# mingfeisun/DeepMimic_mujoco

Hardware: AMD Instinct MI355X
Metric: env-steps/sec (higher is better)
Workload: dtype f64

## Files before the change

deepmimic_mujoco_amd/csrc/slot_kernel.h:

```cpp
#pragma once

#include <cstddef>

#include "env_kernel.h"

namespace dm {

constexpr int SLOTS = 4, SW = 16;
#ifndef DM_SLOT_MAXROWS
#define DM_SLOT_MAXROWS 40
#endif
constexpr int SLOT_MAXROWS = DM_SLOT_MAXROWS, SLOT_MAXLIMROWS = 16, SLOT_MAXCON = 13, SLOT_MAXFRAME = 8, SLOT_MAXCAND = 32, SLOT_BOXSLOTS = 3;
constexpr int SLOT_EXTROWS = SLOT_MAXROWS - 2 * SW;
static_assert(SLOT_EXTROWS == 8 || SLOT_EXTROWS == 0, "the partial third row set holds eight rows (or is absent)");
constexpr int PAIR_PASSES = MAXPAIR / SW;
static_assert(MAXPAIR <= 128 && NG <= 16, "a candidate word holds the pair number in 7 bits and both geom numbers in 4 bits each");
constexpr int DOF_PASSES = (NV + SW - 1) / SW, HINGE_PASSES = (NU + SW - 1) / SW, Q_PASSES = (NQ + SW - 1) / SW, ENT_PASSES = (310 + SW - 1) / SW;

#ifndef DM_SLOT_ASSUME
#define DM_SLOT_ASSUME 31
#endif
#define DM_SLOT_LANE_AT(bit, x) (((DM_SLOT_ASSUME) >> (bit)) & 1 ? dmw::launder_slot_lane(x) : dmw::launder(x))

template <class R>
// ... 815 lines not shown
      dmw::pgs_row3<2 * J + 6>(t3, tsave3, t[0], t[1], nf03, B[J + 3], U[0][J + 3], U[1][J + 3], oh[2 * J + 6]);
      if (J + 4 < next) SlotExtSweep<J + 4, R>::run(U, B, t3, tsave3, t, nf03, oh, next);
    }
  }
};
template <int I, class R>
DM_DEV void slot_assemble_lane(R* ws, const R* fy, R one) {
#pragma unroll
  for (int d = 0; d + 8 <= NV; d += 8) dmw::row_add8<I>(&ws[d], &fy[d], one);
#pragma unroll
  for (int d = NV / 8 * 8; d < NV; d++) dmw::row_fmac_old<I>(ws[d], fy[d], one);
}
template <int J, class R>
struct SlotExtAssemble {
  static DM_DEV void run(R* ws, const R* fy3, R one, int next) {
    if constexpr (J < SLOT_EXTROWS) {
      slot_assemble_lane<2 * J, R>(ws, fy3, one); slot_assemble_lane<2 * J + 2, R>(ws, fy3, one); slot_assemble_lane<2 * J + 4, R>(ws, fy3, one); slot_assemble_lane<2 * J + 6, R>(ws, fy3, one);
      if (J + 4 < next) SlotExtAssemble<J + 4, R>::run(ws, fy3, one, next);
    }
  }
};

template <class R>
DM_DEV void slot_row_setup(const DevModel<R>& M, const SlotShared<R>& s, int r, bool active, RowAcc<R>& ra, R& pos, R& margin, R& dA, R& rscale) {
  const auto& W = s.r1.rw;
  const int code = active ? W.rowi[r] : 0;
  const int type = code & 0xff;
  R w[6] = {0, 0, 0, 0, 0, 0};
  unsigned long long mplus = 0, mminus = 0;
  pos = 0; margin = 0; dA = 0; rscale = 1;
  R w7 = 0;
  if (type == ROW_LIMIT) {
    const int d = (code >> 8) & 0xff;
    w7 = ((code >> 16) & 1) ? R(1) : R(-1);
    pos = W.rowv[r]; dA = M.dof_invw[d]; mplus = 1ull << d;
  } else if (type == ROW_CONTACT) {
    const int ci = (code >> 8) & 0xff, q = (code >> 16) & 0xf, cdim = (code >> 20) & 0xf;
    const R* c = W.con[ci];
    const int cw = W.coni[ci];
    const R* fm = W.frm[(cw >> 8) & 0xff];
    const auto& rec = M.pair_rec[cw & 0xff];
    const R cmu = rec.mu, ctran = rec.tran;
    const int meta = rec.meta;
    R dir[3] = {fm[0], fm[1], fm[2]};
    if (cdim != 1) {
      const R n[3] = {fm[0], fm[1], fm[2]}, t1[3] = {fm[3], fm[4], fm[5]};
      R t2[3];
      cross3(t2, n, t1);
      const R sg = (q & 1) ? -cmu : cmu;
      const R* tg = (q >> 1) ? t2 : t1;
      dir[0] += sg * tg[0]; dir[1] += sg * tg[1]; dir[2] += sg * tg[2];
    }
    cross3(w, c, dir);
    w[3] = dir[0]; w[4] = dir[1]; w[5] = dir[2];
    pos = c[3]; margin = rec.margin;
    dA = cdim == 1 ? ctran : ctran + cmu * cmu * ctran;
    rscale = cdim == 1 ? R(1) : 2 * cmu * cmu;
    mminus = TOPO.chain[meta & 0xff]; mplus = TOPO.chain[(meta >> 8) & 0xff];
  }
  for (int r6 = 0; r6 < 6; r6++) ra.w[r6] = w[r6];
  ra.w7 = w7; ra.w8 = 0; ra.vel = 0; ra.jws = 0;
  ra.plus_lo = (unsigned)mplus; ra.plus_hi = (unsigned)(mplus >> 32); ra.minus_lo = (unsigned)mminus; ra.minus_hi = (unsigned)(mminus >> 32);
}

template <class R, int NS, bool PROF = false>
DM_DEV void slot_constraint(const DevModel<R>& M, SlotShared<R>& s, int sl_in, int lane_in, int nefc, int nmax, int& ovf, const DebugOut* dbg, long long* prof = 0) {
  const int sl = DM_SLOT_LANE_AT(4, sl_in), lane = dmw::launder(lane_in);
  long long pt0 = 0, pt1 = 0, pt_enter = 0;
  if (PROF) { pt0 = dmw::clk(); pt_enter = pt0; }
#define SLOT_STAMP(k) if constexpr (NS == 1) { DM_MARK("slot_constraint_ns1_" #k); } else if constexpr (NS == 2) { DM_MARK("slot_constraint_ns2_" #k); } else { DM_MARK("slot_constraint_ns3_" #k); } if (PROF) { pt1 = dmw::clk(); prof[k] += pt1 - pt0; pt0 = pt1; }
  constexpr bool EXT = NS == 3;
  constexpr int NF = EXT ? 2 : NS;
  constexpr int NC = 16 * NF;
  constexpr int NX = EXT ? SLOT_EXTROWS : 1;
  if constexpr (NS == 1) { DM_MARK("slot_constraint_ns1_rows"); } else if constexpr (NS == 2) { DM_MARK("slot_constraint_ns2_rows"); } else { DM_MARK("slot_constraint_ns3_rows"); }
  R y[NF + 1][NV];
  RowAcc<R> ra[NF];
  bool active[NF];
  R pos[NF], margin[NF], dA[NF], rscale[NF];
#pragma unroll
  for (int k = 0; k < NF; k++) {
    const int r = sl + 16 * k;
    active[k] = r < nefc;
    slot_row_setup(M, s, r, active[k], ra[k], pos[k], margin[k], dA[k], rscale[k]);
  }
  {
    R cur[8];
    dmw::reload_fence();
    slot_load_dof_operands<0>(cur, s);
    SlotRowStep<0, NF, R>::run(y, ra, s, cur);
  }
#pragma unroll
  for (int d = 0; d < NV; d++) y[NF][d] = s.tau[d];
  if (dbg) {
#pragma unroll
    for (int k = 0; k < NF; k++) if (active[k]) {
      double* o = dbg->out + (34 * 34 + 34 * 3 + 42 + 3) + (sl + 16 * k) * (34 + 6);
#pragma unroll
      for (int d = 0; d < NV; d++) o[d] = (double)y[k][d];
    }
  }
  SLOT_STAMP(8)
  R Rr[NF], aref[NF], f[NF];
#pragma unroll
  for (int k = 0; k < NF; k++) {
    const R imp = impedance(M, pos[k] - margin[k]);
    Rr[k] = fmax(R(DM_MINVAL), (1 - imp) * dA[k] / imp);
    if (rscale[k] != R(1)) Rr[k] = fmax(R(DM_MINVAL), rscale[k] * Rr[k]);
    aref[k] = -M.B * ra[k].vel - M.K * imp * (pos[k] - margin[k]);
    const R jar = ra[k].jws - aref[k];
    f[k] = (active[k] && jar < 0) ? -jar / Rr[k] : R(0);
  }
  slot_solve_LT<NF + 1>(y, s.r2.qLD);
#pragma unroll
  for (int d = 0; d < NV; d++) {
    const R sc = s.dsq[d];
#pragma unroll
    for (int k = 0; k <= NF; k++) { y[k][d] *= sc; dmw::pin_value(y[k][d]); }
  }
  if (dbg) {
    R x[NV];
#pragma unroll
    for (int d = 0; d < NV; d++) x[d] = y[NF][d] * s.dsq[d];
    solve_L(x, s.r2.qLD);
    if (sl == 0) {
#pragma unroll
      for (int d = 0; d < NV; d++) dbg->out[34 * 34 + 34 + d] = (double)x[d];
    }
  }
  R bb[NF];
#pragma unroll
  for (int k = 0; k < NF; k++) {
    R acc0 = 0, acc1 = 0;
#pragma unroll
    for (int d = 0; d < NV; d++) { if (d & 1) acc1 += y[k][d] * y[NF][d]; else acc0 += y[k][d] * y[NF][d]; }
    bb[k] = active[k] ? (acc0 + acc1) - aref[k] : R(0);
  }
  R y3[EXT ? NV : 1];
  bool active3 = false;
  R Rr3 = 0, f3 = 0, bb3 = 0;
  if constexpr (EXT) {
    dmw::sync();
    if (sl == 0) {
#pragma unroll
      for (int d = 0; d < NV; d++) s.tau[d] = y[NF][d];
    }
    const int r3 = 2 * SW + (sl >> 1);
    active3 = (sl & 1) == 0 && r3 < nefc;
    RowAcc<R> ra3[1];
    R pos3, margin3, dA3, rscale3;
    slot_row_setup(M, s, r3, active3, ra3[0], pos3, margin3, dA3, rscale3);
    R yy[1][NV];
    {
      R cur[8];
      dmw::reload_fence();
      slot_load_dof_operands<0>(cur, s);
      SlotRowStep<0, 1, R>::run(yy, ra3, s, cur);
    }
    const R imp = impedance(M, pos3 - margin3);
    Rr3 = fmax(R(DM_MINVAL), (1 - imp) * dA3 / imp);
    if (rscale3 != R(1)) Rr3 = fmax(R(DM_MINVAL), rscale3 * Rr3);
    const R aref3 = -M.B * ra3[0].vel - M.K * imp * (pos3 - margin3);
    const R jar = ra3[0].jws - aref3;
    f3 = (active3 && jar < 0) ? -jar / Rr3 : R(0);
    slot_solve_LT<1>(yy, s.r2.qLD);
    dmw::sync();
    R acc0 = 0, acc1 = 0;
#pragma unroll
    for (int d = 0; d < NV; d++) {
      y3[d] = yy[0][d] * s.dsq[d]; dmw::pin_value(y3[d]);
      if (d & 1) acc1 += y3[d] * s.tau[d]; else acc0 += y3[d] * s.tau[d];
    }
    bb3 = active3 ? (acc0 + acc1) - aref3 : R(0);
  }
  R U[EXT ? 2 : 1][NX], B3[NX];
  R diag3 = 1;
  if constexpr (EXT) {
#pragma unroll
    for (int j = 0; j < NX; j++) { U[0][j] = 0; U[1][j] = 0; B3[j] = 0; dmw::pin_value(U[0][j]); dmw::pin_value(U[1][j]); dmw::pin_value(B3[j]); }
    dmw::dpp_settle();
    SlotExtCols<0, R>::run(U, B3, y, y3, nmax - 2 * SW);
    R dg = 1;
#pragma unroll
    for (int j = 0; j < NX; j++) { if (sl == 2 * j) { B3[j] += active3 ? Rr3 : R(0); dg = B3[j]; } }
    diag3 = active3 ? dg : R(1);
    R* y3lds = &s.qd.o.qacc[0];
    if ((sl & 1) == 0) {
#pragma unroll
      for (int d = 0; d < NV; d++) y3lds[d * SLOT_EXTROWS + (sl >> 1)] = y3[d];
    }
  }
  SLOT_STAMP(9)
  R AR[NF][NC];
#pragma unroll
  for (int k = 0; k < NF; k++)
#pragma unroll
    for (int c = 0; c < NC; c++) { AR[k][c] = 0; dmw::pin_value(AR[k][c]); }
  dmw::dpp_settle();
  SlotACols<0, NF, R>::run(AR, y, nmax);
  R diag[NF];
#pragma unroll
  for (int k = 0; k < NF; k++) {
    R dg = 1;
#pragma unroll
    for (int c = 0; c < 16; c++) { if (sl == c) { AR[k][16 * k + c] += active[k] ? Rr[k] : R(0); dg = AR[k][16 * k + c]; } }
    diag[k] = active[k] ? dg : R(1);
  }
  SLOT_STAMP(10)
  typedef decltype(dmw::park(R(0))) ParkedR;
  ParkedR ypark[NF == 2 ? NF : 1][NF == 2 ? NV : 1];
  if constexpr (NF == 2) {
    if constexpr (!EXT) {
      if (sl == 0) {
#pragma unroll
        for (int d = 0; d < NV; d++) s.tau[d] = y[NF][d];
      }
    }
#pragma unroll
    for (int k = 0; k < NF; k++)
#pragma unroll
      for (int d = 0; d < NV; d++) ypark[k][d] = dmw::park(y[k][d]);
#pragma unroll
    for (int k = 0; k < NF; k++)
#pragma unroll
      for (int c = 0; c < NC; c++) dmw::pin_value(AR[k][c]);
    if constexpr (EXT) {
#pragma unroll
      for (int j = 0; j < NX; j++) { dmw::pin_value(U[0][j]); dmw::pin_value(U[1][j]); dmw::pin_value(B3[j]); }
    }
  }
  R ndinv[NF], tb[NF], t[NF];
#pragma unroll
  for (int k = 0; k < NF; k++) { ndinv[k] = active[k] ? R(-1) / diag[k] : R(0); dmw::pin_value(ndinv[k]); tb[k] = bb[k] * ndinv[k]; t[k] = tb[k]; }
  SlotWarm<0, NF, R>::run(AR, t, f, ndinv, nmax);
  R ndinv3 = 0, tb3 = 0;
  if constexpr (EXT) {
    ndinv3 = active3 ? R(-1) / diag3 : R(0); dmw::pin_value(ndinv3);
    tb3 = bb3 * ndinv3;
    dmw::dpp_settle();
    SlotExtWarm<0, R>::run(U, B3, t, f3, ndinv, ndinv3, nmax - 2 * SW);
  }
  {
    R c = 0;
#pragma unroll
    for (int k = 0; k < NF; k++) { const R res = -t[k] * diag[k]; c += active[k] ? f[k] * (R(0.5) * (res - bb[k]) + bb[k]) : R(0); }
    if constexpr (EXT) {
      const R t3 = slot_ext_residual(U, B3, f, diag, f3, tb3, ndinv3, sl);
      const R res = -t3 * diag3;
      c += active3 ? f3 * (R(0.5) * (res - bb3) + bb3) : R(0);
    }
    const R cost = dmw::sum16(c);
    if (cost > 0) {
#pragma unroll
      for (int k = 0; k < NF; k++) { f[k] = 0; t[k] = tb[k]; }
      f3 = 0;
    }
  }
  SLOT_STAMP(11)
  const int maxiter = dmw::uniform(M.iterations);
  R pgs_scale = M.pgs_scale, pgs_tol = M.tolerance, pgs_detect = M.pgs_detect;
  dmw::pin_value(pgs_scale); dmw::pin_value(pgs_tol); dmw::pin_value(pgs_detect);
  int iter = 0;
  bool frozen = nefc == 0 || maxiter <= 0, anybad = false;
  if (frozen) {
#pragma unroll
    for (int k = 0; k < NF; k++) t[k] = 0;
  }
  R oh[16];
#pragma unroll
  for (int i = 0; i < 16; i++) { oh[i] = sl == i ? R(1) : R(0); dmw::pin_value(oh[i]); }
  R nf[NF], nf3 = -f3;
#pragma unroll
  for (int k = 0; k < NF; k++) nf[k] = -f[k];
  R pgs_ntol = -pgs_tol;
  dmw::pin_value(pgs_ntol);
  auto sweep = [&](R& chg, bool& bad) {
    const int nm = dmw::launder_uniform(nmax);
    R tsave[NF];
#pragma unroll
    for (int k = 0; k < NF; k++) tsave[k] = 0;
    SlotSweep<0, NF, R>::run(AR, t, tsave, nf, oh, nm);
    bad = false;
#pragma unroll
    for (int k = 0; k < NF; k++) {
      const R delta = dmw::max_raw(nf[k], tsave[k]);
      const R change = (delta * diag[k]) * (R(0.5) * delta - tsave[k]);
      chg = k == 0 ? change : chg + change;
      nf[k] -= delta; bad = bad || (change > pgs_detect);
    }
    if constexpr (EXT) {
      R fnow[NF];
#pragma unroll
      for (int k = 0; k < NF; k++) fnow[k] = -nf[k];
      const R f3now = -nf3;
      R t3 = slot_ext_residual(U, B3, fnow, diag, f3now, tb3, ndinv3, sl);
      t3 = frozen ? R(0) : t3;
      R tsave3 = 0;
      SlotExtSweep<0, R>::run(U, B3, t3, tsave3, t, nf3, oh, nm - 2 * SW);
      const R delta = dmw::max_raw(nf3, tsave3);
      const R change = (delta * diag3) * (R(0.5) * delta - tsave3);
      nf3 -= delta; chg += change; bad = bad || (change > pgs_detect);
    }
  };
  if (dmw::ballot(!frozen) != 0ull) {
    R chg; bool bad;
    sweep(chg, bad);
    if (!frozen) { iter = 1; anybad = bad; }
    bool more = true;
    while (more) {
      R nfprev[NF], nfprev3 = nf3;
#pragma unroll
      for (int k = 0; k < NF; k++) nfprev[k] = nf[k];
      const R schg = dmw::sum16(chg) * pgs_scale;
      R chg2; bool bad2;
      sweep(chg2, bad2);
      const bool act = !frozen;
      const bool conv = (int)act & ((int)(schg > pgs_ntol) | (int)(iter >= maxiter));
#pragma unroll
      for (int k = 0; k < NF; k++) {
        nf[k] = conv ? nfprev[k] : nf[k];
        t[k] = conv ? R(0) : t[k];
      }
      if constexpr (EXT) nf3 = conv ? nfprev3 : nf3;
      const bool go = (int)act & (int)!conv;
      iter += go ? 1 : 0;
      anybad = (int)anybad | ((int)go & (int)bad2);
      frozen = (int)frozen | (int)conv;
      chg = chg2;
      more = dmw::ballot(!frozen) != 0ull;
      if (PROF) prof[6] += 1;
    }
  }
#pragma unroll
  for (int k = 0; k < NF; k++) f[k] = -nf[k];
  f3 = -nf3;
  if (PROF && NS >= 2) { prof[22] += dmw::clk() - pt0; }
  if (PROF && NS == 3) { prof[27] += dmw::clk() - pt0; }
  SLOT_STAMP(12)
  if (PROF) { prof[14] += nmax; prof[15] += 1; }
  if (dmw::row_ballot(anybad, lane) != 0u) ovf |= 16 | 64;
  if (dbg) {
#pragma unroll
    for (int k = 0; k < NF; k++) if (active[k]) {
      double* o = dbg->out + (34 * 34 + 34 * 3 + 42 + 3) + (sl + 16 * k) * (34 + 6) + 34;
      o[0] = (double)pos[k]; o[1] = (double)margin[k]; o[2] = (double)Rr[k]; o[3] = (double)aref[k]; o[4] = (double)bb[k]; o[5] = (double)f[k];
    }
  }
  R fy3[EXT ? NV : 1];
  if constexpr (EXT) {
    const R* y3lds = &s.qd.o.qacc[0];
    const R f3a = active3 ? f3 : R(0);
#pragma unroll
    for (int d = 0; d < NV; d++) { fy3[d] = ((sl & 1) == 0 ? y3lds[d * SLOT_EXTROWS + (sl >> 1)] : R(0)) * f3a; dmw::pin_value(fy3[d]); }
  }
  if constexpr (NF == 2) {
    dmw::sync();
#pragma unroll
    for (int d = 0; d < NV; d++) y[NF][d] = s.tau[d];
  }
#pragma unroll
  for (int k = 0; k < NF; k++) {
    const R fk = active[k] ? f[k] : R(0);
#pragma unroll
    for (int d = 0; d < NV; d++) { if constexpr (NF == 2) y[k][d] = dmw::unpark(ypark[k][d]); y[k][d] *= fk; dmw::pin_value(y[k][d]); }
  }
  R ws[NV];
#pragma unroll
  for (int d = 0; d < NV; d++) { ws[d] = 0; dmw::pin_value(ws[d]); }
  R one = 1;
  dmw::pin_value(one);
  dmw::dpp_settle();
  SlotAssemble<0, NF, R>::run(ws, y, one, nmax);
  if constexpr (EXT) SlotExtAssemble<0, R>::run(ws, fy3, one, nmax - 2 * SW);
#pragma unroll
  for (int d = 0; d < NV; d++) ws[d] = (ws[d] + y[NF][d]) * s.dsq[d];
  solve_L(ws, s.r2.qLD);
  if (sl == 0) {
#pragma unroll
    for (int d = 0; d < NV; d++) s.qd.o.qacc[d] = ws[d];
    s.solver_iter = iter;
  }
  dmw::sync();
  SLOT_STAMP(13)
  if (PROF && NS >= 2) prof[24] += dmw::clk() - pt_enter;
  if (PROF && NS == 3) prof[26] += dmw::clk() - pt_enter;
#undef SLOT_STAMP
}

#if !defined(DM_WAVE_TESTBENCH)
template <class R, int MAXR>
static __device__ __noinline__ int slot_rows_call(const DevModel<R>* M, SlotShared<R>* s, int sl, int lane, int* ovf) {
  int o = *ovf;
  const int n = slot_rows<R, false, MAXR>(*dmw::in_constant(M), *dmw::in_lds(s), sl, lane, o, (long long*)0);
  *ovf = o;
  return n;
}
#endif

template <class R>
DM_DEV void slot_smooth_solve(SlotShared<R>& s, int sl, const DebugOut* dbg) {
  R x[1][NV];
#pragma unroll
  for (int d = 0; d < NV; d++) x[0][d] = s.tau[d];
  slot_solve_LT<1>(x, s.r2.qLD);
#pragma unroll
  for (int d = 0; d < NV; d++) { x[0][d] *= s.dsq[d]; dmw::pin_value(x[0][d]); }
#pragma unroll
  for (int d = 0; d < NV; d++) x[0][d] = (R(0) + x[0][d]) * s.dsq[d];
  solve_L(x[0], s.r2.qLD);
  if (sl == 0) {
#pragma unroll
    for (int d = 0; d < NV; d++) { s.qd.o.qacc[d] = x[0][d]; if (dbg) dbg->out[34 * 34 + 34 + d] = (double)x[0][d]; }
    s.solver_iter = 0;
  }
  dmw::sync();
}

template <class R, bool PROF = false, bool CARRY = false, int MAXR = 2 * SW>
DM_DEV void slot_forward(const DevModel<R>& M, SlotShared<R>& s, const SlotTables& tb, int sl, int lane, const LaneTopo& lt, R* xip, int& ovf, const DebugOut* dbg, long long* prof = 0) {
  long long t0 = 0, t1 = 0;
  if (PROF) t0 = dmw::clk();
#define SLOT_FSTAMP(k) if (PROF) { t1 = dmw::clk(); prof[k] += t1 - t0; t0 = t1; }
  DM_MARK("slot_kinematics");
  bool skip_kin = false;
  if constexpr (CARRY) {
    skip_kin = dmw::ballot(s.kin_ok() != R(0)) == ~0ull;
    dmw::sync();
    if (sl == 0) s.kin_ok() = R(0);
  }
  if (!skip_kin) slot_kinematics(M, s, sl, lt, xip);
  SLOT_FSTAMP(0)
  if (dbg) { for (int e = sl; e < NV * NV; e += SW) dbg->out[e] = 0; dmw::sync(); }
  DM_MARK("slot_bias");
  slot_bias(M, s, tb, sl, lt);
  SLOT_FSTAMP(1)
  if (dbg) {
    for (int c = 0; c < DOF_PASSES; c++) { const int d = sl + SW * c; if (d < NV) dbg->out[34 * 34 + d] = (double)(-M.dof_damping[d] * s.qvel[d] + s.act[d] - s.tau[d]); }
  }
  DM_MARK("slot_mass_factor");
  slot_mass_matrix<R, PROF>(M, s, tb, sl, lt, dbg, prof);
  SLOT_FSTAMP(2)
  DM_MARK("slot_rows");
  int nefc = 0;
#if !defined(DM_WAVE_TESTBENCH)
  if (!PROF && (M.enable_contact || M.enable_limit)) nefc = slot_rows_call<R, MAXR>(&M, &s, sl, lane, &ovf);
  else
#endif
  if (M.enable_contact || M.enable_limit) nefc = slot_rows<R, PROF, MAXR>(M, s, sl, lane, ovf, prof);
  else { if (sl == 0) { s.nefc = 0; s.ncon = 0; } dmw::sync(); }
  SLOT_FSTAMP(3)
  DM_MARK("slot_constraint");
  const int nmax = rows_max(nefc);
  if (nmax == 0) slot_smooth_solve(s, sl, dbg);
#ifdef DM_FORCE_EXT
  else if (nmax > 0 && MAXR > 2 * SW) slot_constraint<R, MAXR > 2 * SW ? 3 : 2, PROF>(M, s, sl, lane, nefc, nmax > 2 * SW ? nmax : 2 * SW + 1, ovf, dbg, prof);
#endif
  else if (nmax <= 16) slot_constraint<R, 1, PROF>(M, s, sl, lane, nefc, nmax, ovf, dbg, prof);
  else if (nmax <= 2 * SW) { slot_constraint<R, 2, PROF>(M, s, sl, lane, nefc, nmax, ovf, dbg, prof); if (PROF) prof[7] += 1; }
  else if constexpr (MAXR > 2 * SW) { slot_constraint<R, 3, PROF>(M, s, sl, lane, nefc, nmax, ovf, dbg, prof); if (PROF) { prof[7] += 1; prof[25] += 1; } }
  SLOT_FSTAMP(4)
  DM_MARK("slot_forward_end");
#undef SLOT_FSTAMP
  if (dbg) {
    for (int c = 0; c < DOF_PASSES; c++) { const int d = sl + SW * c; if (d < NV) dbg->out[34 * 34 + 68 + d] = (double)s.qd.o.qacc[d]; }
    if (sl < NB - 1) for (int k = 0; k < 3; k++) dbg->out[34 * 34 + 102 + 3 * (sl + 1) + k] = (double)xip[k];
    if (sl == 0) { dbg->out[34 * 34 + 144] = s.nefc; dbg->out[34 * 34 + 145] = s.ncon; dbg->out[34 * 34 + 146] = s.solver_iter; }
  }
}

}
```

deepmimic_mujoco_amd/csrc/wave.h:

```cpp
#pragma once

#if defined(DM_WAVE_TESTBENCH)
#include "wave_testbench.h"
#else
#include <hip/hip_runtime.h>

#define DM_DEV __device__ __forceinline__
#define DM_DEV_NOINLINE __device__ __noinline__
#ifndef DM_NO_STATIC_CALLS
#define DM_STATIC_CALLS 1
#define DM_DEV_CALL64 static __device__ __noinline__
#else
#define DM_DEV_CALL64 __device__ __noinline__
#endif
#define DM_CONSTANT __device__ constexpr

namespace dmw {
DM_DEV int lane() { return (int)(threadIdx.x & 63u); }
DM_DEV void sync() { __builtin_amdgcn_fence(__ATOMIC_SEQ_CST, "wavefront"); __builtin_amdgcn_wave_barrier(); }
DM_DEV void sync_mem() { __syncthreads(); }
DM_DEV unsigned long long ballot(bool p) { return __ballot(p); }
DM_DEV int shfl_i(int v, int src) { return __shfl(v, src, 64); }
DM_DEV double shfl(double v, int src) { return __shfl(v, src, 64); }
DM_DEV float shfl(float v, int src) { return __shfl(v, src, 64); }
DM_DEV double shfl_xor(double v, int m) { return __shfl_xor(v, m, 64); }
DM_DEV float shfl_xor(float v, int m) { return __shfl_xor(v, m, 64); }
DM_DEV int shfl_xor_i(int v, int m) { return __shfl_xor(v, m, 64); }
DM_DEV int shfl_up_i(int v, int d) { return __shfl_up(v, d, 64); }
DM_DEV double bcast(double v, int src) {
  int lo = __double2loint(v), hi = __double2hiint(v);
  lo = __builtin_amdgcn_readlane(lo, src);
  hi = __builtin_amdgcn_readlane(hi, src);
  return __hiloint2double(hi, lo);
}
DM_DEV float bcast(float v, int src) { return __int_as_float(__builtin_amdgcn_readlane(__float_as_int(v), src)); }
DM_DEV int bcast_i(int v, int src) { return __builtin_amdgcn_readlane(v, src); }
template <int CTRL>
DM_DEV double dpp_f64(double v) {
  int lo = __double2loint(v), hi = __double2hiint(v);
  lo = __builtin_amdgcn_update_dpp(0, lo, CTRL, 0xf, 0xf, true);
  hi = __builtin_amdgcn_update_dpp(0, hi, CTRL, 0xf, 0xf, true);
  return __hiloint2double(hi, lo);
}
template <int CTRL>
DM_DEV float dpp_f32(float v) { return __int_as_float(__builtin_amdgcn_update_dpp(0, __float_as_int(v), CTRL, 0xf, 0xf, true)); }
DM_DEV float perm_xor1(float v) { return dpp_f32<0xB1>(v); }
DM_DEV float perm_xor2(float v) { return dpp_f32<0x4E>(v); }
DM_DEV float perm_half_mirror(float v) { return dpp_f32<0x141>(v); }
DM_DEV float perm_row_mirror(float v) { return dpp_f32<0x140>(v); }
DM_DEV double perm_xor1(double v) { return dpp_f64<0xB1>(v); }
DM_DEV double perm_xor2(double v) { return dpp_f64<0x4E>(v); }
DM_DEV double perm_half_mirror(double v) { return dpp_f64<0x141>(v); }
DM_DEV double perm_row_mirror(double v) { return dpp_f64<0x140>(v); }
DM_DEV int uniform(int v) { return __builtin_amdgcn_readfirstlane(v); }
DM_DEV bool uniform(bool v) { return __builtin_amdgcn_readfirstlane((int)v) != 0; }
DM_DEV double rcp_fast(double x) {
  double r = __builtin_amdgcn_rcp(x);
  double e = __builtin_fma(-x, r, 1.0); r = __builtin_fma(e, r, r);
  e = __builtin_fma(-x, r, 1.0); r = __builtin_fma(e, r, r);
  return r;
}
DM_DEV float rcp_fast(float x) { return 1.0f / x; }
DM_DEV void mfma_16x16x4(double a, double b, double (&d)[4]) {
  typedef double v4d __attribute__((ext_vector_type(4)));
  v4d c = {d[0], d[1], d[2], d[3]};
  c = __builtin_amdgcn_mfma_f64_16x16x4f64(a, b, c, 0, 0, 0);
  d[0] = c[0]; d[1] = c[1]; d[2] = c[2]; d[3] = c[3];
}
DM_DEV void mfma_16x16x4(float a, float b, float (&d)[4]) {
  typedef float v4f __attribute__((ext_vector_type(4)));
  v4f c = {d[0], d[1], d[2], d[3]};
  c = __builtin_amdgcn_mfma_f32_16x16x4f32(a, b, c, 0, 0, 0);
  d[0] = c[0]; d[1] = c[1]; d[2] = c[2]; d[3] = c[3];
}
DM_DEV int mfma_row(int lane_id, int v, double) { return (lane_id >> 4) + 4 * v; }
DM_DEV int mfma_row(int lane_id, int v, float) { return 4 * (lane_id >> 4) + v; }
DM_DEV double max_raw(double a, double b) { double r; asm("v_max_f64 %0, %1, %2" : "=v"(r) : "v"(a), "v"(b)); return r; }
DM_DEV float max_raw(float a, float b) { float r; asm("v_max_f32 %0, %1, %2" : "=v"(r) : "v"(a), "v"(b)); return r; }
DM_DEV long long clk() { return (long long)__builtin_readcyclecounter(); }
DM_DEV void sched_fence() { __builtin_amdgcn_sched_barrier(0); }
DM_DEV int pin_zero() { int z = 0; asm volatile("" : "+s"(z)); return z; }
DM_DEV void pin_value(double& v) { asm volatile("" : "+v"(v)); }
DM_DEV void pin_value(float& v) { asm volatile("" : "+v"(v)); }
DM_DEV int launder(int v) { asm volatile("" : "+v"(v)); return v; }
DM_DEV int launder_slot_lane(int v) { asm volatile("" : "+v"(v)); __builtin_assume(v >= 0 && v < 16); return v; }
DM_DEV unsigned long long launder(unsigned long long v) { asm volatile("" : "+v"(v)); return v; }
DM_DEV int launder_uniform(int v) { asm volatile("" : "+s"(v)); return v; }
template <class T> DM_DEV T* uniform_ptr(T* p) {
  const unsigned long long v = (unsigned long long)p;
  const unsigned lo = __builtin_amdgcn_readfirstlane((unsigned)v), hi = __builtin_amdgcn_readfirstlane((unsigned)(v >> 32));
  return (T*)(((unsigned long long)hi << 32) | lo);
}
template <class T> DM_DEV T* in_lds(T* p) {
#if defined(__HIP_DEVICE_COMPILE__)
  __builtin_assume(__builtin_amdgcn_is_shared((const void*)p));
#endif
  return p;
}
template <class T> DM_DEV T* in_global(T* p) {
  __attribute__((address_space(1))) T* g = (__attribute__((address_space(1))) T*)uniform_ptr(p);
  asm volatile("" : "+s"(g));
  return (T*)g;
}
template <class T> DM_DEV const T* in_constant(const T* p) {
  __attribute__((address_space(4))) const T* g = (__attribute__((address_space(4))) const T*)uniform_ptr(p);
  asm volatile("" : "+s"(g));
  return (const T*)g;
}
template <class T> DM_DEV T* launder_uniform_ptr(T* p) { asm volatile("" : "+s"(p)); return p; }
DM_DEV void reload_fence() { asm volatile("" ::: "memory"); }
DM_DEV void lds_sub(bool pred, double* p, double v) { if (pred) __hip_atomic_fetch_add(p, -v, __ATOMIC_RELAXED, __HIP_MEMORY_SCOPE_WORKGROUP); }
DM_DEV void lds_sub(bool pred, float* p, float v) { if (pred) __hip_atomic_fetch_add(p, -v, __ATOMIC_RELAXED, __HIP_MEMORY_SCOPE_WORKGROUP); }
template <int I> DM_DEV double row_bcast(double v) {
  long long x = __double_as_longlong(v);
  x = __builtin_amdgcn_update_dpp(0ll, x, 0x150 + I, 0xf, 0xf, true);
  return __longlong_as_double(x);
}
template <int I> DM_DEV float row_bcast(float v) { return __int_as_float(__builtin_amdgcn_update_dpp(0, __float_as_int(v), 0x150 + I, 0xf, 0xf, true)); }
template <int I> DM_DEV int row_bcast_i(int v) { return __builtin_amdgcn_update_dpp(0, v, 0x150 + I, 0xf, 0xf, true); }
template <int I> DM_DEV void row_fmac(double& acc, double x, double y) {
  asm volatile("s_nop 1\n\tv_fmac_f64_dpp %0, %1, %2 row_newbcast:%3 row_mask:0xf bank_mask:0xf" : "+v"(acc) : "v"(x), "v"(y), "n"(I));
}
template <int I> DM_DEV void row_fmac(float& acc, float x, float y) { acc += row_bcast<I>(x) * y; }
template <int I> DM_DEV void row_fmac_old(double& acc, double x, double y) {
  asm volatile("s_nop 1\n\tv_fmac_f64_dpp %0, %1, %2 row_newbcast:%3 row_mask:0xf bank_mask:0xf" : "+v"(acc) : "v"(x), "v"(y), "n"(I));
}
template <int I> DM_DEV void row_fmac_old(float& acc, float x, float y) { acc += row_bcast<I>(x) * y; }
#define DM_FMAC_DPP(acc, x, y) "v_fmac_f64_dpp " acc ", " x ", " y " row_newbcast:%18 row_mask:0xf bank_mask:0xf\n\t"
template <int I> DM_DEV void row_fmac8(double& acc0, double& acc1, const double* x, const double* y) {
  asm volatile("s_nop 1\n\t" DM_FMAC_DPP("%0", "%2", "%10") DM_FMAC_DPP("%1", "%3", "%11") DM_FMAC_DPP("%0", "%4", "%12") DM_FMAC_DPP("%1", "%5", "%13")
               DM_FMAC_DPP("%0", "%6", "%14") DM_FMAC_DPP("%1", "%7", "%15") DM_FMAC_DPP("%0", "%8", "%16") DM_FMAC_DPP("%1", "%9", "%17")
               : "+v"(acc0), "+v"(acc1)
               : "v"(x[0]), "v"(x[1]), "v"(x[2]), "v"(x[3]), "v"(x[4]), "v"(x[5]), "v"(x[6]), "v"(x[7]),
                 "v"(y[0]), "v"(y[1]), "v"(y[2]), "v"(y[3]), "v"(y[4]), "v"(y[5]), "v"(y[6]), "v"(y[7]), "n"(I));
}
#undef DM_FMAC_DPP
#define DM_FMAC_DPP(acc, x) "v_fmac_f64_dpp " acc ", " x ", %16 row_newbcast:%17 row_mask:0xf bank_mask:0xf\n\t"
template <int I> DM_DEV void row_add8(double* a, const double* x, double one) {
  asm volatile("s_nop 1\n\t" DM_FMAC_DPP("%0", "%8") DM_FMAC_DPP("%1", "%9") DM_FMAC_DPP("%2", "%10") DM_FMAC_DPP("%3", "%11")
               DM_FMAC_DPP("%4", "%12") DM_FMAC_DPP("%5", "%13") DM_FMAC_DPP("%6", "%14") DM_FMAC_DPP("%7", "%15")
               : "+v"(a[0]), "+v"(a[1]), "+v"(a[2]), "+v"(a[3]), "+v"(a[4]), "+v"(a[5]), "+v"(a[6]), "+v"(a[7])
               : "v"(x[0]), "v"(x[1]), "v"(x[2]), "v"(x[3]), "v"(x[4]), "v"(x[5]), "v"(x[6]), "v"(x[7]), "v"(one), "n"(I));
}
#undef DM_FMAC_DPP
template <int I> DM_DEV void row_fmac8(float& acc0, float& acc1, const float* x, const float* y) { for (int k = 0; k < 8; k++) { if (k & 1) acc1 += row_bcast<I>(x[k]) * y[k]; else acc0 += row_bcast<I>(x[k]) * y[k]; } }
template <int I> DM_DEV void row_add8(float* a, const float* x, float one) { for (int k = 0; k < 8; k++) a[k] += row_bcast<I>(x[k]) * one; }
template <int I> DM_DEV void pgs_row(double& t, double& tsave, double nf0, double a, double onehot) {
  double delta;
  asm volatile("v_max_f64 %0, %3, %1\n\tv_fma_f64 %2, %5, %1, %2\n\ts_nop 0\n\tv_fmac_f64_dpp %1, %0, %4 row_newbcast:%6 row_mask:0xf bank_mask:0xf"
               : "=&v"(delta), "+v"(t), "+v"(tsave) : "v"(nf0), "v"(a), "v"(onehot), "n"(I));
}
template <int I> DM_DEV void pgs_row2(double& t_own, double& tsave_own, double& t_other, double nf0, double a_own, double a_other, double onehot) {
  double delta;
  asm volatile("v_max_f64 %0, %4, %1\n\tv_fma_f64 %2, %7, %1, %2\n\ts_nop 0\n\tv_fmac_f64_dpp %1, %0, %5 row_newbcast:%8 row_mask:0xf bank_mask:0xf\n\t"
               "v_fmac_f64_dpp %3, %0, %6 row_newbcast:%8 row_mask:0xf bank_mask:0xf"
               : "=&v"(delta), "+v"(t_own), "+v"(tsave_own), "+v"(t_other) : "v"(nf0), "v"(a_own), "v"(a_other), "v"(onehot), "n"(I));
}
template <int I> DM_DEV void pgs_row3(double& t3, double& tsave3, double& t0, double& t1, double nf0, double b, double u0, double u1, double onehot) {
  double delta;
  asm volatile("v_max_f64 %0, %5, %1\n\tv_fma_f64 %2, %9, %1, %2\n\ts_nop 0\n\tv_fmac_f64_dpp %1, %0, %6 row_newbcast:%10 row_mask:0xf bank_mask:0xf\n\t"
               "v_fmac_f64_dpp %3, %0, %7 row_newbcast:%10 row_mask:0xf bank_mask:0xf\n\tv_fmac_f64_dpp %4, %0, %8 row_newbcast:%10 row_mask:0xf bank_mask:0xf"
               : "=&v"(delta), "+v"(t3), "+v"(tsave3), "+v"(t0), "+v"(t1) : "v"(nf0), "v"(b), "v"(u0), "v"(u1), "v"(onehot), "n"(I));
}
template <int I> DM_DEV void pgs_row3(float& t3, float& tsave3, float& t0, float& t1, float nf0, float b, float u0, float u1, float onehot) {
  const float d = max_raw(nf0, t3); tsave3 += onehot * t3; const float bc = row_bcast<I>(d); t3 += bc * b; t0 += bc * u0; t1 += bc * u1;
}
#define DM_PGS1(D, A, OH, I) "v_max_f64 " D ", %3, %0\n\tv_fma_f64 %1, " OH ", %0, %1\n\ts_nop 0\n\tv_fmac_f64_dpp %0, " D ", " A " row_newbcast:" I " row_mask:0xf bank_mask:0xf\n\t"
template <int I0> DM_DEV void pgs_rows4(double& t, double& tsave, double nf0, const double* a, const double* oh) {
  double d;
  asm volatile(DM_PGS1("%2", "%4", "%8", "%12") DM_PGS1("%2", "%5", "%9", "%13") DM_PGS1("%2", "%6", "%10", "%14") DM_PGS1("%2", "%7", "%11", "%15")
               : "+v"(t), "+v"(tsave), "=&v"(d)
               : "v"(nf0), "v"(a[0]), "v"(a[1]), "v"(a[2]), "v"(a[3]), "v"(oh[0]), "v"(oh[1]), "v"(oh[2]), "v"(oh[3]), "n"(I0), "n"(I0 + 1), "n"(I0 + 2), "n"(I0 + 3));
}
#undef DM_PGS1
template <int I0> DM_DEV void pgs_rows4_2(double& t_own, double& tsave_own, double& t_other, double nf0, const double* a_own, const double* a_other, const double* oh) {
  double d0, d1;
  asm volatile(
      "v_max_f64 %3, %5, %0\n\tv_fma_f64 %1, %14, %0, %1\n\ts_nop 0\n\tv_fmac_f64_dpp %0, %3, %6 row_newbcast:%18 row_mask:0xf bank_mask:0xf\n\t"
      "v_max_f64 %4, %5, %0\n\tv_fma_f64 %1, %15, %0, %1\n\tv_fmac_f64_dpp %2, %3, %10 row_newbcast:%18 row_mask:0xf bank_mask:0xf\n\tv_fmac_f64_dpp %0, %4, %7 row_newbcast:%19 row_mask:0xf bank_mask:0xf\n\t"
      "v_max_f64 %3, %5, %0\n\tv_fma_f64 %1, %16, %0, %1\n\tv_fmac_f64_dpp %2, %4, %11 row_newbcast:%19 row_mask:0xf bank_mask:0xf\n\tv_fmac_f64_dpp %0, %3, %8 row_newbcast:%20 row_mask:0xf bank_mask:0xf\n\t"
      "v_max_f64 %4, %5, %0\n\tv_fma_f64 %1, %17, %0, %1\n\tv_fmac_f64_dpp %2, %3, %12 row_newbcast:%20 row_mask:0xf bank_mask:0xf\n\tv_fmac_f64_dpp %0, %4, %9 row_newbcast:%21 row_mask:0xf bank_mask:0xf\n\t"
      "s_nop 0\n\tv_fmac_f64_dpp %2, %4, %13 row_newbcast:%21 row_mask:0xf bank_mask:0xf"
      : "+v"(t_own), "+v"(tsave_own), "+v"(t_other), "=&v"(d0), "=&v"(d1)
      : "v"(nf0), "v"(a_own[0]), "v"(a_own[1]), "v"(a_own[2]), "v"(a_own[3]), "v"(a_other[0]), "v"(a_other[1]), "v"(a_other[2]), "v"(a_other[3]),
        "v"(oh[0]), "v"(oh[1]), "v"(oh[2]), "v"(oh[3]), "n"(I0), "n"(I0 + 1), "n"(I0 + 2), "n"(I0 + 3));
}
template <int I> DM_DEV void pgs_row(float& t, float& tsave, float nf0, float a, float onehot) { const float d = max_raw(nf0, t); tsave += onehot * t; t += row_bcast<I>(d) * a; }
template <int I> DM_DEV void pgs_row2(float& t_own, float& tsave_own, float& t_other, float nf0, float a_own, float a_other, float onehot) {
  const float d = max_raw(nf0, t_own); tsave_own += onehot * t_own; const float b = row_bcast<I>(d); t_own += b * a_own; t_other += b * a_other;
}
template <int I0> DM_DEV void pgs_rows4(float& t, float& tsave, float nf0, const float* a, const float* oh) {
  pgs_row<I0>(t, tsave, nf0, a[0], oh[0]); pgs_row<I0 + 1>(t, tsave, nf0, a[1], oh[1]); pgs_row<I0 + 2>(t, tsave, nf0, a[2], oh[2]); pgs_row<I0 + 3>(t, tsave, nf0, a[3], oh[3]);
}
template <int I0> DM_DEV void pgs_rows4_2(float& t_own, float& tsave_own, float& t_other, float nf0, const float* a_own, const float* a_other, const float* oh) {
  pgs_row2<I0>(t_own, tsave_own, t_other, nf0, a_own[0], a_other[0], oh[0]); pgs_row2<I0 + 1>(t_own, tsave_own, t_other, nf0, a_own[1], a_other[1], oh[1]);
  pgs_row2<I0 + 2>(t_own, tsave_own, t_other, nf0, a_own[2], a_other[2], oh[2]); pgs_row2<I0 + 3>(t_own, tsave_own, t_other, nf0, a_own[3], a_other[3], oh[3]);
}
DM_DEV void dpp_settle() { asm volatile("s_nop 4"); }
struct Parked { int lo, hi; };
DM_DEV Parked park(double v) {
  Parked p;
  asm volatile("v_accvgpr_write_b32 %0, %2\n\tv_accvgpr_write_b32 %1, %3" : "=a"(p.lo), "=a"(p.hi) : "v"(__double2loint(v)), "v"(__double2hiint(v)));
  return p;
}
DM_DEV double unpark(const Parked& p) {
  int lo, hi;
  asm volatile("v_accvgpr_read_b32 %0, %2\n\tv_accvgpr_read_b32 %1, %3" : "=v"(lo), "=v"(hi) : "a"(p.lo), "a"(p.hi));
  return __hiloint2double(hi, lo);
}
struct ParkedF { int x; };
DM_DEV ParkedF park(float v) { ParkedF p; asm volatile("v_accvgpr_write_b32 %0, %1" : "=a"(p.x) : "v"(__float_as_int(v))); return p; }
DM_DEV float unpark(const ParkedF& p) { int x; asm volatile("v_accvgpr_read_b32 %0, %1" : "=v"(x) : "a"(p.x)); return __int_as_float(x); }
DM_DEV int global_counter_next(int* p) { return atomicAdd(p, 1); }
DM_DEV unsigned row_ballot(bool p, int lane_id) { return (unsigned)((__ballot(p) >> (lane_id & 48)) & 0xffffull); }
}
#endif

namespace dmw {
DM_DEV double sum8(double v) { v += perm_xor1(v); v += perm_xor2(v); v += perm_half_mirror(v); return v; }
DM_DEV double sum16(double v) { v = sum8(v); v += perm_row_mirror(v); return v; }
DM_DEV double wave_sum(double v) {
  v = sum16(v);
  return ((bcast(v, 0) + bcast(v, 16)) + bcast(v, 32)) + bcast(v, 48);
}
#if !defined(DM_WAVE_TESTBENCH)
DM_DEV float sum8(float v) { v += perm_xor1(v); v += perm_xor2(v); v += perm_half_mirror(v); return v; }
DM_DEV float sum16(float v) { v = sum8(v); v += perm_row_mirror(v); return v; }
DM_DEV float wave_sum(float v) {
  v = sum16(v);
  return ((bcast(v, 0) + bcast(v, 16)) + bcast(v, 32)) + bcast(v, 48);
}
#endif
DM_DEV int wave_exclusive_scan(int v, int lane_id, int* total) {
  const unsigned long long below = (1ull << lane_id) - 1ull;
  int pre = 0, tot = 0;
#pragma unroll
  for (int b = 0; b < 5; b++) {
    const unsigned long long m = ballot(((v >> b) & 1) != 0);
    pre += __builtin_popcountll(m & below) << b;
    tot += __builtin_popcountll(m) << b;
  }
  *total = tot;
  return pre;
}
}
```

Baseline: 20.64 million.

## Unroll PGS convergence loop to two sweeps per wave-vote round

The default PGS loop now runs two speculative sweeps per iteration, with a third sweep overlapping the convergence check. It does the two change reductions together in an interleaved cross-lane sum and resolves convergence for both steps at once, rolling back to the matching saved state. The aim is to halve the number of wave ballots and serialized reduction latencies per convergence check. In exchange, slots that converge mid-pair do extra wasted sweeps, register pressure rises from holding two saved force sets, and the old loop is kept behind a macro.

```diff
diff --git a/deepmimic_mujoco_amd/csrc/slot_kernel.h b/deepmimic_mujoco_amd/csrc/slot_kernel.h
--- a/deepmimic_mujoco_amd/csrc/slot_kernel.h
+++ b/deepmimic_mujoco_amd/csrc/slot_kernel.h
@@ -1141,6 +1141,7 @@
       nf3 -= delta; chg += change; bad = bad || (change > pgs_detect);
     }
   };
+#if defined(DM_PGS_ONE_SWEEP)
   if (dmw::ballot(!frozen) != 0ull) {
     R chg; bool bad;
     sweep(chg, bad);
@@ -1170,6 +1171,48 @@
       if (PROF) prof[6] += 1;
     }
   }
+#else
+  if (dmw::ballot(!frozen) != 0ull) {
+    R chg; bool bad;
+    sweep(chg, bad);
+    if (!frozen) { iter = 1; anybad = bad; }
+    bool more = true;
+    while (more) {
+      R nfa[NF], nfa3 = nf3;
+#pragma unroll
+      for (int k = 0; k < NF; k++) nfa[k] = nf[k];
+      R chgb; bool badb;
+      sweep(chgb, badb);
+      R nfb[NF], nfb3 = nf3;
+#pragma unroll
+      for (int k = 0; k < NF; k++) nfb[k] = nf[k];
+      R sa = chg, sb = chgb;
+      dmw::sum16x2(sa, sb);
+      sa *= pgs_scale; sb *= pgs_scale;
+      R chgc; bool badc;
+      sweep(chgc, badc);
+      const bool act = !frozen;
+      const bool conva = (int)act & ((int)(sa > pgs_ntol) | (int)(iter >= maxiter));
+      const bool goa = (int)act & (int)!conva;
+      const int iterb = iter + (goa ? 1 : 0);
+      const bool convb = (int)goa & ((int)(sb > pgs_ntol) | (int)(iterb >= maxiter));
+      const bool gob = (int)goa & (int)!convb;
+      const bool conv = (int)conva | (int)convb;
+#pragma unroll
+      for (int k = 0; k < NF; k++) {
+        nf[k] = conva ? nfa[k] : convb ? nfb[k] : nf[k];
+        t[k] = conv ? R(0) : t[k];
+      }
+      if constexpr (EXT) nf3 = conva ? nfa3 : convb ? nfb3 : nf3;
+      iter = iterb + (gob ? 1 : 0);
+      anybad = (int)anybad | ((int)goa & (int)badb) | ((int)gob & (int)badc);
+      frozen = (int)frozen | (int)conv;
+      chg = chgc;
+      more = dmw::ballot(!frozen) != 0ull;
+      if (PROF) prof[6] += 2;
+    }
+  }
+#endif
 #pragma unroll
   for (int k = 0; k < NF; k++) f[k] = -nf[k];
   f3 = -nf3;
diff --git a/deepmimic_mujoco_amd/csrc/wave.h b/deepmimic_mujoco_amd/csrc/wave.h
--- a/deepmimic_mujoco_amd/csrc/wave.h
+++ b/deepmimic_mujoco_amd/csrc/wave.h
@@ -219,6 +219,12 @@
 namespace dmw {
 DM_DEV double sum8(double v) { v += perm_xor1(v); v += perm_xor2(v); v += perm_half_mirror(v); return v; }
 DM_DEV double sum16(double v) { v = sum8(v); v += perm_row_mirror(v); return v; }
+template <class T> DM_DEV void sum16x2(T& a, T& b) {
+  a += perm_xor1(a); b += perm_xor1(b);
+  a += perm_xor2(a); b += perm_xor2(b);
+  a += perm_half_mirror(a); b += perm_half_mirror(b);
+  a += perm_row_mirror(a); b += perm_row_mirror(b);
+}
 DM_DEV double wave_sum(double v) {
   v = sum16(v);
   return ((bcast(v, 0) + bcast(v, 16)) + bcast(v, 32)) + bcast(v, 48);
```

New measurement: 20.72 million (median of 6 runs). About the same (+0.4%).
